# OllieBoyne/sslap

Hardware: AMD Instinct MI355X
Metric: Medges/s (bid-phase CSR nnz/s) + solve ms, N=200k d=0.1% sparse LAP (higher is better)
Workload: dtype f64

## Files before the change

### sslap_amd/csrc/device_common.hpp

```cpp
#pragma once
#include <hip/hip_runtime.h>
#include <stdint.h>

#include <type_traits>

namespace misslap {

constexpr int kWave = 64;
constexpr int kPosNone = 0x7fffffff;
constexpr int kTailMax = 512;

constexpr int kErrNegativeBid = 1;
constexpr int kErrRowsUnsorted = 2;
constexpr int kErrRowGap = 4;
constexpr int kErrNonFinite = 8;
constexpr int kErrColNegative = 16;
constexpr int kErrLdsBase = 32;
constexpr int kErrTooMany = 64;
constexpr int kErrPriceFell = 128;

struct Ctl {
    int K;
    int nholes;
    int nleft;
// ... 149 lines not shown
}
__device__ __forceinline__ double readlane_f64(double v, int l) {
    const int lo = __builtin_amdgcn_readlane(__double2loint(v), l);
    const int hi = __builtin_amdgcn_readlane(__double2hiint(v), l);
    return __hiloint2double(hi, lo);
}

#define MISSLAP_WAVE_MAX_STEP(T, EXCH) \
    {                                  \
        const T o = EXCH;              \
        v = o > v ? o : v;             \
    }
__device__ __forceinline__ int wave_max_i32(int v) {
    MISSLAP_WAVE_MAX_STEP(int, __builtin_amdgcn_mov_dpp(v, kDppXor1, 0xF, 0xF, true))
    MISSLAP_WAVE_MAX_STEP(int, __builtin_amdgcn_mov_dpp(v, kDppXor2, 0xF, 0xF, true))
    MISSLAP_WAVE_MAX_STEP(int, __builtin_amdgcn_mov_dpp(v, kDppHalfMirror, 0xF, 0xF, true))
    MISSLAP_WAVE_MAX_STEP(int, __builtin_amdgcn_mov_dpp(v, kDppMirror, 0xF, 0xF, true))
    MISSLAP_WAVE_MAX_STEP(int, (dpp_i32<kDppBcast15, 0xA>(v)))
    MISSLAP_WAVE_MAX_STEP(int, (dpp_i32<kDppBcast31, 0xC>(v)))
    return __builtin_amdgcn_readlane(v, 63);
}
__device__ __forceinline__ double wave_max_f64(double v) {
    v = __builtin_fmax(v, dpp_f64<kDppXor1>(v));
    v = __builtin_fmax(v, dpp_f64<kDppXor2>(v));
    v = __builtin_fmax(v, dpp_f64<kDppHalfMirror>(v));
    v = __builtin_fmax(v, dpp_f64<kDppMirror>(v));
    v = __builtin_fmax(v, (dpp_f64<kDppBcast15, 0xA>(v)));
    v = __builtin_fmax(v, (dpp_f64<kDppBcast31, 0xC>(v)));
    return readlane_f64(v, 63);
}
#undef MISSLAP_WAVE_MAX_STEP

struct Top2 {
    double v, w;
    int g;
};
__device__ __forceinline__ Top2 top2_wave_reduce(const Top2 &x) {
    Top2 r;
    r.v = wave_max_f64(x.v);
    r.g = wave_max_i32(x.v == r.v ? x.g : -1);
    r.w = wave_max_f64(x.g == r.g ? x.w : x.v);
    return r;
}

struct __attribute__((aligned(16))) PriceRec {
    double price;
    int owner;
    int ostart;
};

__device__ __forceinline__ int lane_id() { return threadIdx.x & (kWave - 1); }
__device__ __forceinline__ unsigned long long lanemask_lt() {
    return (1ull << lane_id()) - 1ull;
}

constexpr int kCandLanes = 32;
constexpr int kCandMax = 30;
constexpr int kCandMin = 24;
constexpr int kCandRowMax = 4 * kWave;

template <int CTRL>
__device__ __forceinline__ int dppf_i32(int v) {
    return __builtin_amdgcn_mov_dpp(v, CTRL, 0xF, 0xF, true);
}
template <int CTRL>
__device__ __forceinline__ double dppf_f64(double v) {
    return __hiloint2double(dppf_i32<CTRL>(__double2hiint(v)), dppf_i32<CTRL>(__double2loint(v)));
}
__device__ __forceinline__ double half_max_f64(double v) {
    v = __builtin_fmax(v, dppf_f64<kDppXor1>(v));
    v = __builtin_fmax(v, dppf_f64<kDppXor2>(v));
    v = __builtin_fmax(v, dppf_f64<kDppHalfMirror>(v));
    v = __builtin_fmax(v, dppf_f64<kDppMirror>(v));
    v = __builtin_fmax(v, (dpp_f64<kDppBcast15, 0xA>(v)));
    return v;
}
__device__ __forceinline__ int half_max_i32(int v) {
    v = max(v, dppf_i32<kDppXor1>(v));
    v = max(v, dppf_i32<kDppXor2>(v));
    v = max(v, dppf_i32<kDppHalfMirror>(v));
    v = max(v, dppf_i32<kDppMirror>(v));
    v = max(v, (dpp_i32<kDppBcast15, 0xA>(v)));
    return v;
}

__device__ __forceinline__ double slot_cost(const int2 &s) { return (double)__int_as_float(s.y); }
__device__ __forceinline__ double slot_cost(const Slot64 &s) { return s.c; }
__device__ __forceinline__ double slot_cost_at(const int2 &s, int sl) {
    return (double)__int_as_float(__builtin_amdgcn_readlane(s.y, sl));
}
__device__ __forceinline__ double slot_cost_at(const Slot64 &s, int sl) { return readlane_f64(s.c, sl); }
template <class Slot>
struct LineIO;
template <>
struct LineIO<int2> {
    static __device__ __forceinline__ int2 load(const int2 *cand, const double *, size_t idx) { return cand[idx]; }
    static __device__ __forceinline__ int2 make(int x, int y) { return make_int2(x, y); }
};
template <>
struct LineIO<Slot64> {
    static __device__ __forceinline__ Slot64 load(const int2 *cand, const double *cost, size_t idx) {
        const int2 s = cand[idx];
        Slot64 r;
        r.x = s.x;
        r.y = s.y;
        r.c = cost[idx];
        return r;
    }
    static __device__ __forceinline__ Slot64 make(int x, int y) {
        Slot64 r;
        r.x = x;
        r.y = y;
        r.c = 0.0;
        return r;
    }
};

struct CandBid {
    bool hit;
    unsigned long long key;
    int obj;
    int prev, pstart;
    int len;
};

struct RecSource {
    const PriceRec *rec;
    __device__ __forceinline__ PriceRec get(int col) const { return rec[col]; }
};
struct PriceSource {
    const double *price;
    __device__ __forceinline__ PriceRec get(int col) const {
        PriceRec r;
        r.price = price[col];
        r.owner = -1;
        r.ostart = 0;
        return r;
    }
};

template <class Slot, class Src>
__device__ __forceinline__ PriceRec cand_gather2(const Slot slot, const bool act0, const bool act1, const Src &src) {
    const int lane = lane_id(), l32 = lane & (kCandLanes - 1);
    const bool active = lane < kCandLanes ? act0 : act1;
    const bool is_cand = active & (l32 >= 1) & (l32 <= kCandMax) & (slot.x >= 0);
    return src.get(is_cand ? slot.x : 0);
}
template <class Slot, class Early, class S = NoStamp>
__device__ __forceinline__ void cand_eval2_r(Slot &slot, const PriceRec r, const bool act0, const bool act1,
                                             const double eps, CandBid (&out)[2], int &err, Early &&early,
                                             const S &stamp = S(), int *alive = nullptr);
template <class Slot, class Src, class Early, class S = NoStamp>
__device__ __forceinline__ void cand_eval2(Slot &slot, const bool act0, const bool act1, const Src &src,
                                           const double eps, CandBid (&out)[2], int &err, Early &&early,
                                           const S &stamp = S(), int *alive = nullptr) {
    stamp(1);
    const PriceRec r = cand_gather2(slot, act0, act1, src);
    stamp(2);
    cand_eval2_r(slot, r, act0, act1, eps, out, err, early, stamp, alive);
}
template <class Slot, class Early, class S>
__device__ __forceinline__ void cand_eval2_r(Slot &slot, const PriceRec r, const bool act0, const bool act1,
                                             const double eps, CandBid (&out)[2], int &err, Early &&early,
                                             const S &stamp, int *alive) {
    const int lane = lane_id(), l32 = lane & (kCandLanes - 1);
    const double ninf = -__builtin_huge_val();
// ... 381 lines not shown
```

### sslap_amd/csrc/host_rounds.hpp

```cpp
#pragma once

namespace {
void begin_phase(misslap_solver *h) {
    if (h->cand != nullptr && !h->lines_dropped && (double)h->eps < h->lines_safe_eps) h->lines_dropped = true;
    h->phases_run += 1;
    h->phases_with_lines += h->lines_live() ? 1 : 0;
}

RoundArgs round_args(misslap_solver *h) {
    RoundArgs a;
    a.ctl = h->ctl;
    a.row_ptr = h->row_ptr;
    a.price = h->price;
    a.rec = h->rec;
    a.p2o = h->p2o;
    a.o2p = h->o2p;
    a.U = h->U;
    a.bid_key = h->bid_key;
    a.bid_obj = h->bid_obj;
    a.bid_rec = h->bid_rec;
    a.best_key = h->best_key;
    a.best_pos = h->best_pos;
    a.cnt = h->cnt;
    a.hole_list = h->hole_list;
// ... 355 lines not shown
    if (h->round_small) {
        h->round_small = false;
        h->K_exact = false;
        MISSLAP_LAUNCH(h, k_round_small, (F_k_round_small), 1024, dim3(1), dim3(1024), a);
        HIP_TRY(hipGetLastError());
        return MISSLAP_OK;
    }
    h->K_exact = false;
    h->round_ordered = false;
    if ((h->world == 1 || h->K_ub < h->shard_min_K) && (long long)h->K_ub * h->apply_bidders_ratio <= h->n_cols)
        MISSLAP_LAUNCH(h, k_apply_bidders, (F_k_apply_bidders), 256, dim3(blocks_for(h->K_ub, 256)), dim3(256), a);
    else
        MISSLAP_LAUNCH(h, k_apply, (F_k_apply), 256, dim3(blocks_for(h->n_cols, 256)), dim3(256), a);
    if (h->K_ub <= kCompactSmallMax) {
        MISSLAP_LAUNCH(h, k_compact_small, (F_k_compact_small), 1024, dim3(1), dim3(1024), a);
    } else {
        const int cb = blocks_for(h->K_ub, kChunk);
        MISSLAP_LAUNCH(h, k_compact_count, (F_k_compact_count), 256, dim3(cb), dim3(256), a);
        MISSLAP_LAUNCH(h, k_compact_scatter, (F_k_compact_scatter), 256, dim3(cb), dim3(256), a);
        MISSLAP_LAUNCH(h, k_compact_fill, (F_k_compact_fill), 256, dim3(blocks_for(h->K_ub, 256)), dim3(256), a);
    }
    HIP_TRY(hipGetLastError());
    return MISSLAP_OK;
}

int launch_tail(misslap_solver *h) {
    if (h->thr <= 0) return MISSLAP_OK;
    h->ctl_fresh = false;
    h->untouched = false;
    const long long long_after = std::max<long long>(kLongRowsAfterTailRoundsMin, h->n_rows / 64);
    if (h->long_rows_later && h->tail_rounds_host >= long_after) {
        h->long_rows = true;
        h->long_rows_later = false;
    }
    TailArgs a;
    a.ctl = h->ctl;
    a.row_ptr = h->row_ptr;
    a.price = h->price;
    a.rec = h->rec;
    a.p2o = h->p2o;
    a.o2p = h->o2p;
    a.U = h->U;
    const bool lines = h->lines_live();
    a.cand = lines ? h->cand : nullptr;
    a.cand64 = lines ? h->cand64 : nullptr;
    a.round_budget = h->long_rows && lines && h->line_maintenance ? h->tail_round_budget
                     : h->long_rows_later                            ? (int)std::min<long long>(std::max<long long>(long_after, 1), 1 << 30)
                                                                     : 0;
    if (a.round_budget == 0 || a.round_budget > h->tail_launch_rounds) a.round_budget = h->tail_launch_rounds;
    a.thr = h->thr;
    a.eps = h->eps;
    ProfRec *pr = nullptr;
    if (h->profile) {
        pr = prof_next(h, 1);
        if (!pr) return fail(MISSLAP_ERR_HIP, "hipEventCreate failed");
        HIP_TRY(hipEventRecord(pr->start, h->stream));
    }
    const EdgesF32 e32{h->edges32};
    const EdgesF64 e64{h->col, h->val64};
    const int long_max = !(lines && h->line_maintenance && h->long_rows) ? 0 : (h->max_row_len <= 256 * kLongPer ? 256 : 512) * kLongPer;
    const int min_alive_long = kLongRowMinAlive;
    const bool in_batch = h->batch != nullptr;
    if (in_batch) h->batch->hold_next = true;
#define MISSLAP_LAUNCH_TAIL(E, ED)                                                                                       \
    do {                                                                                                                 \
        if (lines && h->line_maintenance)                                                                                \
            MISSLAP_LAUNCH(h, k_refresh_lines<E>, (F_k_refresh_lines<E>), kBidBlock,                                     \
                           dim3(blocks_for((h->n_rows + 1) / 2, kBidBlock / kWave)), dim3(kBidBlock), round_args(h), ED, \
                           (int)kCandMaintenanceMin, long_max, min_alive_long);                                          \
        if (lines && h->line_maintenance && h->long_rows) {                                                              \
            if (h->max_row_len <= 256 * kLongPer)                                                                        \
                MISSLAP_LAUNCH(h, (k_refresh_long<E, 256>), (F_k_refresh_long<E, 256>), 256, dim3(blocks_for(h->n_rows, 1)), \
                               dim3(256), round_args(h), ED);                                                            \
            else                                                                                                         \
                MISSLAP_LAUNCH(h, (k_refresh_long<E, 512>), (F_k_refresh_long<E, 512>), 512, dim3(blocks_for(h->n_rows, 1)), \
                               dim3(512), round_args(h), ED);                                                            \
        }                                                                                                                \
        if (h->K_ub > kTeamMax || in_batch)                                                                              \
            MISSLAP_LAUNCH(h, (k_tail<E, 2 * kTailMax>), (F_k_tail<E, 2 * kTailMax, false>), 2 * kTailMax, dim3(1),      \
                           dim3(2 * kTailMax), a, ED);                                                                   \
        if ((h->K_ub > 2 || in_batch) && lines)                                                                          \
            MISSLAP_LAUNCH(h, (k_tail<E, 2 * kTailMax, true>), (F_k_tail<E, 2 * kTailMax, true>), 2 * kTailMax, dim3(1), \
                           dim3(2 * kTailMax), a, ED);                                                                   \
        if (lines) MISSLAP_LAUNCH(h, (k_tail<E, 2 * kWave>), (F_k_tail<E, 2 * kWave, false>), 2 * kWave, dim3(1),        \
                                  dim3(2 * kWave), a, ED);                                                               \
        else MISSLAP_LAUNCH(h, (k_tail<E, kTailMax>), (F_k_tail<E, kTailMax, false>), kTailMax, dim3(1), dim3(kTailMax), a, ED); \
    } while (0)
    if (h->f32) MISSLAP_LAUNCH_TAIL(EdgesF32, e32);
    else MISSLAP_LAUNCH_TAIL(EdgesF64, e64);
#undef MISSLAP_LAUNCH_TAIL
    if (pr) HIP_TRY(hipEventRecord(pr->stop, h->stream));
    h->live_valid = !h->live_off && h->live_dev != nullptr;
    MISSLAP_LAUNCH(h, k_sync_from_rec, (F_k_sync_from_rec), 256, dim3(blocks_for(h->n_cols, 256)), dim3(256), h->ctl,
                   (const PriceRec *)h->rec, h->price, h->o2p, h->p2o, (const int *)h->U, h->n_cols,
                   (h->cand != nullptr && !h->lines_dropped) ? 1 : 0, h->live_valid ? h->live_dev : (unsigned long long *)nullptr,
                   ++h->ticket);
    HIP_TRY(hipGetLastError());
    h->phase_fresh = false;
    if (h->tail_nits0 < 0) h->tail_nits0 = h->h_ctl->nits;
    return MISSLAP_OK;
}

int check_lanes(const misslap_solver *h) {
    if (!h->tiled_ok) return 0;
    const int *shp = kTiledShapes[h->tiled_shape];
    return (shp[3] == 2 && shp[4] == kTileColsHalf) ? shp[6] : 0;
}
#define MISSLAP_FOR_CHECK_LANES(X) X(4) X(8) X(16)
#define MISSLAP_CHECK_KERNEL(GL) k_bid_tiled<1024, 4, 2, 2, kTileColsHalf, 3, 0, GL, 1, 1>
#define MISSLAP_CHECK_KERNEL_FMT(GL, FMT) k_bid_tiled<1024, 4, 2, 2, kTileColsHalf, 3, 0, GL, 1, 1, FMT>

size_t final_pass_grid_max(size_t n_rows, int n_cus) {
    const size_t per_wg_min = (size_t)((1024 - 64 * 3) / 16) * 4;
    return std::max<size_t>((n_rows + per_wg_min - 1) / per_wg_min, (size_t)n_cus);
}
int launch_rows_gather(misslap_solver *h, float eps, const FinalOut &fo, int n_rows, int *n_blocks = nullptr) {
    const int grid = blocks_for(n_rows, 4);
    if (n_blocks) *n_blocks = grid;
    if (h->f32) {
        EdgesF32 ed{h->edges32};
        MISSLAP_LAUNCH(h, k_ece<EdgesF32>, (F_k_ece<EdgesF32>), 256, dim3(grid), dim3(256), h->ctl, ed, (const int *)h->row_ptr,
                       (const double *)h->price, (const int *)h->p2o, n_rows, eps, fo);
    } else {
        EdgesF64 ed{h->col, h->val64};
        MISSLAP_LAUNCH(h, k_ece<EdgesF64>, (F_k_ece<EdgesF64>), 256, dim3(grid), dim3(256), h->ctl, ed, (const int *)h->row_ptr,
                       (const double *)h->price, (const int *)h->p2o, n_rows, eps, fo);
    }
    HIP_TRY(hipGetLastError());
    return MISSLAP_OK;
}
int launch_rows_all(misslap_solver *h, float eps, const FinalOut &fo, int *n_blocks = nullptr) {
    const int gl = check_lanes(h);
    if (!gl) return launch_rows_gather(h, eps, fo, h->n_rows, n_blocks);
    RoundArgs a = round_args(h);
    a.eps = eps;
    a.launch_edges = nullptr;
    TiledArgs ta{h->tiled, h->tcol, h->seg4, h->T, 0, h->n_tiled,
                 nullptr, nullptr, h->ovf_ptr, h->ovf_q, h->ovf_cap, nullptr, nullptr, h->n_rows, nullptr, fo};
    const int groups = (1024 - 64 * 3) / gl, per_wg_max = groups * 4;
    long long grid = ((long long)h->n_rows + per_wg_max - 1) / per_wg_max;
    const long long spread = std::min<long long>(h->n_cus, ((long long)h->n_rows + groups - 1) / groups);
    if (grid < spread) grid = spread;
    if (fo.fin && grid > h->fin_slots_n) return fail(MISSLAP_ERR_STATE, "final pass: grid %lld exceeds its result slots (%d)", grid, h->fin_slots_n);
    if (n_blocks) *n_blocks = (int)grid;
    const size_t lds = tiled_lds_bytes(kTileColsHalf);
    if (h->tiled_fmt == 0) {
        switch (gl) {
#define X(GL) \
    case GL: MISSLAP_LAUNCH_PLAIN(h, (MISSLAP_CHECK_KERNEL(GL)), dim3((unsigned)grid), dim3(1024), lds, a, ta); break;
            MISSLAP_FOR_CHECK_LANES(X)
#undef X
        }
    } else {
        switch (h->tiled_fmt * 100 + gl) {
#define X(FMT, GL) \
    case FMT * 100 + GL: MISSLAP_LAUNCH_PLAIN(h, (MISSLAP_CHECK_KERNEL_FMT(GL, FMT)), dim3((unsigned)grid), dim3(1024), lds, a, ta); break;
            MISSLAP_FOR_FMT_LANES(X)
#undef X
        }
    }
    HIP_TRY(hipGetLastError());
    return MISSLAP_OK;
}

int run_ece(misslap_solver *h, float eps, int *ok) {
    int rc = read_status(h);
    if (rc) return rc;
    if (h->h_ctl->K > 0) {
// ... 48 lines not shown
```

### sslap_amd/csrc/kernels_tail.hpp

```cpp
#pragma once
#include "device_common.hpp"

namespace misslap {

struct TailArgs {
    Ctl *ctl;
    const int *row_ptr;
    double *price;
    PriceRec *rec;
    int *p2o;
    int *o2p;
    int *U;
    int2 *cand;
    double *cand64;
    int thr;
    int round_budget;
    float eps;
};

constexpr int kHashSize = 2048;

__device__ __forceinline__ unsigned long long readlane_u64(unsigned long long v, int l) {
    const int lo = __builtin_amdgcn_readlane((int)(unsigned)(v & 0xffffffffull), l);
    const int hi = __builtin_amdgcn_readlane((int)(unsigned)(v >> 32), l);
// ... 190 lines not shown
    K = pi != -1;
    nits += r;
#ifdef MISSLAP_TAIL_STAMP
    if (lane == 0) {
        for (int k = 1; k <= 6; ++k) a.ctl->dbg[5 + k] += sacc[k];
    }
#endif
}

template <class E>
__device__ __forceinline__ void tail_solo_mode(const TailArgs &a, const E &ed, int *sU, int *sStart, int &K,
                                               long long &nits, const long long max_iter, const double eps,
                                               TailStats &st) {
    const int lane = lane_id();
    int pi[2], ps[2];
    pi[0] = __builtin_amdgcn_readfirstlane(sU[0]);
    ps[0] = __builtin_amdgcn_readfirstlane(sStart[0]);
    pi[1] = K > 1 ? __builtin_amdgcn_readfirstlane(sU[1]) : -1;
    ps[1] = K > 1 ? __builtin_amdgcn_readfirstlane(sStart[1]) : 0;
    if (K == 1) {
        tail_chain_mode(a, ed, pi[0], ps[0], K, nits, max_iter, eps, st);
        if (lane == 0) {
            sU[0] = pi[0];
            sU[1] = -1;
            sStart[0] = ps[0];
        }
        return;
    }
    TwoFetch<E> tf;
    tf.slot = cand_no_line<typename E::Slot>();
    request_two(a, ed, pi[0], ps[0], pi[1], ps[1], tf);
#ifdef MISSLAP_TAIL_STAMP_SOLO
    unsigned long long sacc[8] = {0, 0, 0, 0, 0, 0, 0, 0}, sprev = __builtin_amdgcn_s_memtime();
    const CycleStamp stamp{sacc, &sprev, true};
#else
    const NoStamp stamp;
#endif
    for (;;) {
        CandBid b[2];
        CandBuildArgs bd;
        int bd_person;
        int sp[2] = {-2, -2};
        bid_two(a, ed, pi, ps, tf, eps, b, bd, bd_person, st, [&](const CandBid(&w)[2]) {
            sp[0] = pi[0] >= 0 ? w[0].prev : -1;
            sp[1] = pi[1] >= 0 ? w[1].prev : -1;
            request_two(a, ed, sp[0], 0, sp[1], 0, tf);
        }, stamp);
        stamp.light(5);
        nits += 1;
        bool win0 = true, win1 = pi[1] >= 0;
        if (win1 && b[0].obj == b[1].obj) {
            if (b[1].key > b[0].key) win0 = false;
            else win1 = false;
        }
        if (lane == 0) {
            if (win0) apply_winner(a, pi[0], ps[0], b[0].obj, b[0].prev, b[0].key);
            if (win1) apply_winner(a, pi[1], ps[1], b[1].obj, b[1].prev, b[1].key);
        }
        if (win0) {
            pi[0] = b[0].prev;
            ps[0] = b[0].pstart;
        }
        if (win1) {
            pi[1] = b[1].prev;
            ps[1] = b[1].pstart;
        }
        if (pi[0] == -1 && pi[1] != -1) {
            pi[0] = pi[1];
            ps[0] = ps[1];
            pi[1] = -1;
        }
        K = (pi[0] != -1) + (pi[1] != -1);
        const bool done = K <= 1 || nits >= max_iter;
        if (!done && (sp[0] != pi[0] || sp[1] != pi[1])) request_two(a, ed, pi[0], ps[0], pi[1], ps[1], tf);
        if (bd_person >= 0) tail_build(a, bd_person, bd, eps, st);
        stamp.light(6);
        if (done) break;
    }
    if (K == 1 && nits < max_iter) tail_chain_mode(a, ed, pi[0], ps[0], K, nits, max_iter, eps, st);
#ifdef MISSLAP_TAIL_STAMP_SOLO
    if (lane == 0)
        for (int k = 1; k <= 6; ++k) a.ctl->dbg[5 + k] += sacc[k];
#endif
    if (lane == 0) {
        sU[0] = pi[0];
        sU[1] = pi[1];
        sStart[0] = ps[0];
        sStart[1] = ps[1];
    }
}

constexpr int kTeamMax = 16;
constexpr int kTeamTab = 64;
__device__ __forceinline__ void tail_barrier_lds() { asm volatile("s_waitcnt lgkmcnt(0)\n\ts_barrier" ::: "memory"); }

template <class E>
__device__ __forceinline__ void tail_team_mode(const TailArgs &a, const E &ed, int *sU, int *sStart, int &K,
                                               long long &nits, const long long max_iter, const double eps,
                                               TailStats &st) {
    const int lane = lane_id(), wave = __builtin_amdgcn_readfirstlane(threadIdx.x >> 6);
    static_assert(kTeamMax <= 2 * (kTailMax / kWave) && kTeamMax <= kWave, "two list slots per wavefront");
    __shared__ unsigned long long tKey[2][kTeamMax];
    __shared__ int tObj[2][kTeamMax], tPrev[2][kTeamMax], tPst[2][kTeamMax], tU[2][kTeamMax], tS[2][kTeamMax];
    __shared__ int wTab[kTailMax / kWave][kTeamTab];
    const int n0 = 2 * wave;
    int pi[2], ps[2];
#pragma unroll
    for (int X = 0; X < 2; ++X) {
        pi[X] = n0 + X < K ? __builtin_amdgcn_readfirstlane(sU[min(n0 + X, kTailMax - 1)]) : -1;
        ps[X] = n0 + X < K ? __builtin_amdgcn_readfirstlane(sStart[min(n0 + X, kTailMax - 1)]) : 0;
    }
    wTab[wave][lane & (kTeamTab - 1)] = -1;
    TwoFetch<E> tf;
    tf.slot = cand_no_line<typename E::Slot>();
    if (n0 < K) request_two(a, ed, pi[0], ps[0], pi[1], ps[1], tf);
    __syncthreads();
#ifdef MISSLAP_TAIL_STAMP_TEAM
    unsigned long long sacc[8] = {0, 0, 0, 0, 0, 0, 0, 0}, sprev = __builtin_amdgcn_s_memtime();
    const CycleStamp stamp{sacc, &sprev, wave == 0};
#else
    const NoStamp stamp;
#endif
    int par = 0;
    for (;;) {
        int sp[2] = {-2, -2};
        CandBuildArgs bd;
        int bd_person = -1;
        stamp.light(0);
        if (n0 < K) {
            CandBid b[2];
            bid_two(a, ed, pi, ps, tf, eps, b, bd, bd_person, st, [&](const CandBid(&w)[2]) {
                sp[0] = pi[0] >= 0 ? w[0].prev : -1;
                sp[1] = pi[1] >= 0 ? w[1].prev : -1;
                request_two(a, ed, sp[0], 0, sp[1], 0, tf);
            });
            if (lane == 0) {
#pragma unroll
                for (int X = 0; X < 2; ++X)
                    if (pi[X] >= 0) {
                        tKey[par][n0 + X] = b[X].key;
                        tObj[par][n0 + X] = b[X].obj;
                        tPrev[par][n0 + X] = b[X].prev;
                        tPst[par][n0 + X] = b[X].pstart;
                        tU[par][n0 + X] = pi[X];
                        tS[par][n0 + X] = ps[X];
                    }
            }
        }
        stamp.light(1);
        tail_barrier_lds();
        stamp.light(2);
        {
            const bool act = lane < K;
            const int ls = min(lane, kTeamMax - 1);
            const unsigned long long lkey = act ? tKey[par][ls] : 0ull;
            const int lobj = act ? tObj[par][ls] : (-2 - lane);
            const int lprev = act ? tPrev[par][ls] : 0, lpst = act ? tPst[par][ls] : 0;
            int u = act ? tU[par][ls] : -1;
            int sx = act ? tS[par][ls] : 0;
            int hs = 0;
            bool dup = false;
            if (act) {
                hs = (int)(((unsigned)lobj * 2654435761u) >> 26) & (kTeamTab - 1);
                for (;;) {
                    const int old = atomicCAS(&wTab[wave][hs], -1, lobj);
                    if (old == -1) break;
// ... 1 lines not shown
                        dup = true;
                        break;
                    }
                    hs = (hs + 1) & (kTeamTab - 1);
                }
            }
            const bool contested = __any(dup);
            if (act && !dup) wTab[wave][hs] = -1;
            const bool ends = __any(act && lprev == -1);
#ifdef MISSLAP_TAIL_STAMP_TEAM
            if (threadIdx.x == 0) sacc[5] += (!contested && !ends), sacc[6] += contested, sacc[7] += 1;
#endif
            if (!contested && !ends) {
                if (act && n0 < K) apply_winner(a, u, sx, lobj, lprev, lkey);
#pragma unroll
                for (int X = 0; X < 2; ++X) {
                    const int w = __builtin_amdgcn_readlane(lprev, min(n0 + X, kWave - 1));
                    const int ws = __builtin_amdgcn_readlane(lpst, min(n0 + X, kWave - 1));
                    pi[X] = n0 + X < K ? w : -1;
                    ps[X] = n0 + X < K ? ws : 0;
                }
            } else {
                bool lose = false;
                for (int m = 0; m < K; ++m) {
                    const int om = __builtin_amdgcn_readlane(lobj, m);
                    const bool same = (om == lobj) && (m != lane);
                    if (__any(same)) {
                        const unsigned long long km = readlane_u64(lkey, m);
                        lose |= same && (km > lkey || (km == lkey && m < lane));
                    }
                }
                const bool won = act && !lose;
                if (won && n0 < K) apply_winner(a, u, sx, lobj, lprev, lkey);
                u = won ? lprev : u;
                sx = won ? lpst : sx;
                const unsigned long long kmask = (1ull << K) - 1ull;
                const unsigned long long holes = __ballot(act && u == -1) & kmask;
                const int Kn = K - __popcll(holes);
                const unsigned long long lmask = (1ull << Kn) - 1ull;
                unsigned long long hl = holes & lmask;
                unsigned long long mv = ~holes & ~lmask & kmask;
                while (hl) {
                    const int hk = __ffsll((long long)hl) - 1, mk = __ffsll((long long)mv) - 1;
                    const int mu = __builtin_amdgcn_readlane(u, mk), ms = __builtin_amdgcn_readlane(sx, mk);
                    if (lane == hk) {
                        u = mu;
                        sx = ms;
                    }
                    hl &= hl - 1;
                    mv &= mv - 1;
                }
                K = Kn;
#pragma unroll
                for (int X = 0; X < 2; ++X) {
                    pi[X] = n0 + X < K ? __builtin_amdgcn_readlane(u, min(n0 + X, kWave - 1)) : -1;
                    ps[X] = n0 + X < K ? __builtin_amdgcn_readlane(sx, min(n0 + X, kWave - 1)) : 0;
                }
            }
        }
        stamp.light(3);
        par ^= 1;
        nits += 1;
        const bool done = K <= 2 || nits >= max_iter;
        if (!done && n0 < K && (sp[0] != pi[0] || sp[1] != pi[1]))
            request_two(a, ed, pi[0], ps[0], pi[1], ps[1], tf);
        if (bd_person >= 0) tail_build(a, bd_person, bd, eps, st);
        stamp.light(4);
        if (done) break;
    }
#ifdef MISSLAP_TAIL_STAMP_TEAM
    if (threadIdx.x == 0)
        for (int k = 1; k <= 6; ++k) a.ctl->dbg[5 + k] += sacc[k];
#endif
    if (lane < 2 && n0 + lane < kTeamMax) {
        sU[n0 + lane] = lane == 0 ? pi[0] : pi[1];
        sStart[n0 + lane] = lane == 0 ? ps[0] : ps[1];
    }
    __syncthreads();
}

constexpr int kPipeTab = 4096;
__device__ __forceinline__ int pipe_hash(int obj) { return (int)(((unsigned)obj * 2654435761u) >> 20); }
static_assert((1 << 12) == kPipeTab, "pipe_hash keeps the top 12 bits");
__device__ __forceinline__ void patch_rec(PriceRec &r, const bool take, const PriceRec &nw) {
    r.price = take ? nw.price : r.price;
    r.owner = take ? nw.owner : r.owner;
    r.ostart = take ? nw.ostart : r.ostart;
}
struct __attribute__((aligned(16))) PipeSlot {
    PriceRec rec;
    int4 aux;
};
struct __attribute__((aligned(16))) PipeLds {
    PipeSlot slot[2][kTeamMax];
    int dirty[2];
    int pad[2];
    int tab[kPipeTab];
};

__device__ __forceinline__ void touch_slot(const int2 &s) { asm volatile("" ::"v"(s.x), "v"(s.y)); }
__device__ __forceinline__ void touch_slot(const Slot64 &s) { asm volatile("" ::"v"(s.x), "v"(s.y), "v"(s.c)); }

template <class E>
__device__ __forceinline__ bool tail_team1_pipe(const TailArgs &a, const E &ed, int *sU, int *sStart, int &K,
                                                long long &nits, const long long max_iter, const double eps,
                                                TailStats &st) {
    const int lane = lane_id(), l32 = lane & (kCandLanes - 1);
    const int wave = __builtin_amdgcn_readfirstlane(threadIdx.x >> 6);
    __shared__ PipeLds L;
    const RecSource src{a.rec};
    const bool cls = (lane >= 1) & (lane <= kCandMax);
    const int n0 = wave;
    int pi = n0 < K ? __builtin_amdgcn_readfirstlane(sU[min(n0, kTailMax - 1)]) : -1;
    int ps = n0 < K ? __builtin_amdgcn_readfirstlane(sStart[min(n0, kTailMax - 1)]) : 0;
    for (int h = threadIdx.x; h < kPipeTab; h += blockDim.x) L.tab[h] = -1;
    if (threadIdx.x < 2) L.dirty[threadIdx.x] = -1;
    typename E::Slot slot = cand_no_line<typename E::Slot>();
    auto request = [&](int person) { slot = line_of<E>(a, person, l32); };
    if (n0 < K) request(pi);
    __syncthreads();
#ifdef MISSLAP_TAIL_STAMP_TEAM
    unsigned long long sacc[8] = {0, 0, 0, 0, 0, 0, 0, 0}, sprev = __builtin_amdgcn_s_memtime();
    const CycleStamp stamp{sacc, &sprev, wave == 0};
#else
    const NoStamp stamp;
#endif
    const int rmax = round_limit(nits, max_iter);
    int r = 0;
    int par = 0;
    const int ls = min(lane, kTeamMax - 1);
    PriceRec grec = PriceRec{0.0, -1, 0};
    bool have_g = false;
    for (;;) {
        if (n0 >= K) {
            if (lane == 0) {
                sU[n0] = -1;
                sStart[n0] = 0;
            }
            tail_barrier_lds();
            nits += r;
            return true;
        }
        int sp = -2;
        CandBid b;
        b.hit = false;
        stamp.light(0);
        if (!have_g) grec = cand_gather1(slot, cls, src);
#ifdef MISSLAP_TAIL_STAMP_TEAM
        asm volatile("s_waitcnt vmcnt(0)" ::: "memory");
        stamp.light(1);
#endif
        cand_eval1_r(slot, grec, cls, eps, b, st.bad_hi, [&](const CandBid &w) {
            sp = w.prev;
            request(sp);
        });
        if (!b.hit) {
            CandBuildArgs bd;
            const typename E::Raw none[4] = {};
            const int e = a.row_ptr[pi + 1 + lane_zero()];
            wave_bid_full<E, RecSource, true, false>(ed, src, ps, e, none, eps, b, bd, st.err);
            st.misses += 1;
            st.miss_edges += (unsigned long long)b.len;
            if (bd.want) tail_build(a, pi, bd, eps, st);
        }
        st.edges += (unsigned long long)b.len;
        st.bids += 1;
        stamp.light(2);
        if (lane == 0) {
            const int old = atomicExch(&L.tab[pipe_hash(b.obj)], r);
            PriceRec mine;
            mine.price = key_to_bid(b.key);
// ... 8 lines not shown
        stamp.light(4);
        {
            const int dflag = L.dirty[par];
            const PriceRec lrec = L.slot[par][ls].rec;
            const int lobj = L.slot[par][ls].aux.x;
#ifdef MISSLAP_TAIL_STAMP_TEAM
            asm volatile("s_waitcnt lgkmcnt(0)" ::: "memory");
            stamp.light(5);
#endif
            if (__builtin_amdgcn_readfirstlane(dflag) != r) {
                have_g = sp == b.prev;
                if (have_g) {
                    touch_slot(slot);
                    if (lane < K) a.rec[lobj] = lrec;
                    grec = cand_gather1(slot, cls, src);
                } else {
                    if (lane < K) a.rec[lobj] = lrec;
                }
                pi = b.prev;
                ps = b.pstart;
            } else {
                have_g = false;
                const bool act = lane < K;
                const int4 laux = L.slot[par][ls].aux;
                const unsigned long long lkey = act ? bid_to_key(lrec.price) : 0ull;
                const int lo = act ? laux.x : (-2 - lane);
                const int lprev = act ? laux.y : 0, lpst = act ? laux.z : 0;
                int u = act ? lrec.owner : -1;
                int sx = act ? lrec.ostart : 0;
                bool lose = false;
                for (int m = 0; m < K; ++m) {
                    const int om = __builtin_amdgcn_readlane(lo, m);
                    const bool same = (om == lo) && (m != lane);
                    if (__any(same)) {
                        const unsigned long long km = readlane_u64(lkey, m);
                        lose |= same && (km > lkey || (km == lkey && m < lane));
                    }
                }
                const bool won = act && !lose;
                if (won) apply_winner(a, u, sx, lo, lprev, lkey);
                u = won ? lprev : u;
                sx = won ? lpst : sx;
                const unsigned long long kmask = (1ull << K) - 1ull;
                const unsigned long long holes = __ballot(act && u == -1) & kmask;
                const int Kn = K - __popcll(holes);
                const unsigned long long lmask = (1ull << Kn) - 1ull;
                unsigned long long hl = holes & lmask;
                unsigned long long mv = ~holes & ~lmask & kmask;
                while (hl) {
                    const int hk = __ffsll((long long)hl) - 1, mk = __ffsll((long long)mv) - 1;
                    const int mu = __builtin_amdgcn_readlane(u, mk), ms = __builtin_amdgcn_readlane(sx, mk);
                    if (lane == hk) {
                        u = mu;
                        sx = ms;
                    }
                    hl &= hl - 1;
                    mv &= mv - 1;
                }
                K = Kn;
                pi = n0 < K ? __builtin_amdgcn_readlane(u, min(n0, kWave - 1)) : -1;
                ps = n0 < K ? __builtin_amdgcn_readlane(sx, min(n0, kWave - 1)) : 0;
            }
        }
        par ^= 1;
        r += 1;
        const bool done = K <= 2 || r >= rmax;
        if (!done && n0 < K && sp != pi) request(pi);
        stamp.light(6);
        if (done) break;
    }
    nits += r;
#ifdef MISSLAP_TAIL_STAMP_TEAM
    if (threadIdx.x == 0)
        for (int k = 1; k <= 6; ++k) a.ctl->dbg[5 + k] += sacc[k];
#endif
    if (lane == 0 && n0 < kTeamMax) {
        sU[n0] = pi;
        sStart[n0] = ps;
    }
    __syncthreads();
    return false;
}

template <class E>
__device__ __forceinline__ void tail_duo_pipe(const TailArgs &a, const E &ed, int *sU, int *sStart, int &K,
                                              long long &nits, const long long max_iter, const double eps,
                                              TailStats &st) {
    const int lane = lane_id(), l32 = lane & (kCandLanes - 1);
    const int w = __builtin_amdgcn_readfirstlane(threadIdx.x >> 6);
    const int o = w ^ 1;
    __shared__ PipeSlot D[2][2];
    const RecSource src{a.rec};
    const bool cls = (lane >= 1) & (lane <= kCandMax);
    int me = __builtin_amdgcn_readfirstlane(sU[w]), mys = __builtin_amdgcn_readfirstlane(sStart[w]);
    typename E::Slot slot = cand_no_line<typename E::Slot>();
    auto request = [&](int person) { slot = line_of<E>(a, person, l32); };
    request(me);
    tail_barrier_lds();
#ifdef MISSLAP_TAIL_STAMP_DUO
    unsigned long long sacc[8] = {0, 0, 0, 0, 0, 0, 0, 0}, sprev = __builtin_amdgcn_s_memtime();
    const CycleStamp stamp{sacc, &sprev, w == 0};
#else
    const NoStamp stamp;
#endif
    const int rmax = round_limit(nits, max_iter);
    int r = 0;
    PriceRec grec = PriceRec{0.0, -1, 0};
    bool have_g = false;
    int par = 0;
    bool pend = false;
    PriceRec prec = PriceRec{0.0, -1, 0};
    int pobj = 0;
    auto flush_store = [&]() {
        if (pend) {
            if (lane < 2) a.rec[pobj] = prec;
            pend = false;
        }
    };
    for (;;) {
        int sp = -2;
        CandBid b;
        b.hit = false;
        stamp.light(0);
        if (!have_g) {
            flush_store();
            grec = cand_gather1(slot, cls, src);
        }
        cand_eval1_r(slot, grec, cls, eps, b, st.bad_hi, [&](const CandBid &x) {
            sp = x.prev;
            request(sp);
        });
        if (!b.hit) {
            flush_store();
            CandBuildArgs bd;
            const typename E::Raw none[4] = {};
            const int e = a.row_ptr[me + 1 + lane_zero()];
            wave_bid_full<E, RecSource, true, false>(ed, src, mys, e, none, eps, b, bd, st.err);
            st.misses += 1;
            st.miss_edges += (unsigned long long)b.len;
            if (bd.want) tail_build(a, me, bd, eps, st);
            b.hit = false;
        }
        flush_store();
        st.edges += (unsigned long long)b.len;
        st.bids += 1;
        stamp.light(1);
        PriceRec mine;
        mine.price = key_to_bid(b.key);
        mine.owner = me;
        mine.ostart = mys;
        if (lane == 0) {
            D[par][w].rec = mine;
            D[par][w].aux = make_int4(b.obj, b.prev, b.pstart, 0);
        }
        have_g = b.hit && b.prev >= 0;
        if (have_g) grec = cand_gather1(slot, cls, src);
        stamp.light(2);
        tail_barrier_lds();
        stamp.light(3);
        const PriceRec orec = D[par][o].rec;
        const int4 oaux = D[par][o].aux;
        r += 1;
        const int unclean = __builtin_amdgcn_readfirstlane((int)(oaux.x == b.obj) | (int)(oaux.y < 0)) | (int)(b.prev < 0);
        if (!unclean) {
            if (have_g) {
                const int c = slot.x;
                patch_rec(grec, c == b.obj, mine);
                patch_rec(grec, c == oaux.x, orec);
            }
            pend = true;
            prec = mine;
            patch_rec(prec, lane == 1, orec);
            pobj = lane == 1 ? oaux.x : b.obj;
            me = b.prev;
            mys = b.pstart;
        } else {
            const unsigned long long okey = bid_to_key(readlane_f64(orec.price, 0));
            const int oobj = __builtin_amdgcn_readfirstlane(oaux.x), oprev = __builtin_amdgcn_readfirstlane(oaux.y);
            const int opst = __builtin_amdgcn_readfirstlane(oaux.z);
            const int ome = __builtin_amdgcn_readfirstlane(orec.owner), omys = __builtin_amdgcn_readfirstlane(orec.ostart);
            int pi[2], ps[2];
            pi[0] = w ? ome : me, pi[1] = w ? me : ome;
            ps[0] = w ? omys : mys, ps[1] = w ? mys : omys;
            const unsigned long long key0 = w ? okey : b.key, key1 = w ? b.key : okey;
            const int obj0 = w ? oobj : b.obj, obj1 = w ? b.obj : oobj;
            const int prev0 = w ? oprev : b.prev, prev1 = w ? b.prev : oprev;
            const int pst0 = w ? opst : b.pstart, pst1 = w ? b.pstart : opst;
            bool win0 = true, win1 = true;
            if (obj0 == obj1) {
                if (key1 > key0) win0 = false;
                else win1 = false;
            }
            if (lane == 0) {
                if (win0) apply_winner(a, pi[0], ps[0], obj0, prev0, key0);
                if (win1) apply_winner(a, pi[1], ps[1], obj1, prev1, key1);
            }
            if (win0) {
                pi[0] = prev0;
                ps[0] = pst0;
            }
            if (win1) {
                pi[1] = prev1;
                ps[1] = pst1;
            }
            if (pi[0] == -1 && pi[1] != -1) {
                pi[0] = pi[1];
                ps[0] = ps[1];
                pi[1] = -1;
            }
            K = (pi[0] != -1) + (pi[1] != -1);
            me = w ? pi[1] : pi[0];
            mys = w ? ps[1] : ps[0];
            have_g = false;
        }
        stamp.light(4);
        par ^= 1;
        const bool done = K <= 1 || r >= rmax;
        if (!done && sp != me) request(me);
        stamp.light(5);
        if (done) break;
    }
    flush_store();
    nits += r;
#ifdef MISSLAP_TAIL_STAMP_DUO
    if (w == 0 && lane == 0)
        for (int k = 1; k <= 5; ++k) a.ctl->dbg[5 + k] += sacc[k];
#endif
    if (lane == 0) {
        sU[w] = me;
        sStart[w] = mys;
    }
    tail_barrier_lds();
}

template <class E, int kThreads, bool kTeamOnly>
__device__ __forceinline__ void k_tail_body(TailArgs a, E ed) {
    static_assert(!kTeamOnly || (kThreads == 2 * kTailMax && kThreads / kWave == kTeamMax), "one slot per wavefront");
    constexpr bool kBlockOnly = kThreads > kTailMax && !kTeamOnly;
    constexpr bool kDuoOnly = kThreads == 2 * kWave;
    static_assert(!kDuoOnly || !kTeamOnly, "roles are exclusive");
    __shared__ int sU[kTailMax];
    __shared__ unsigned long long sKey[kTailMax];
    __shared__ int sObj[kTailMax];
    __shared__ int sPrev[kTailMax];
    __shared__ int sStart[kTailMax];
    __shared__ int sPst[kTailMax];
    __shared__ int sList[kTailMax];
    __shared__ int hObj[kHashSize];
    __shared__ unsigned long long hKey[kHashSize];
    __shared__ int hPos[kHashSize];
    __shared__ int sCnt[3][kThreads / kWave];
    __shared__ int sK, sMissCnt;
    __shared__ long long sNits;

    Ctl *ctl = a.ctl;
    const int t = threadIdx.x, lane = t & 63, wave = t >> 6;
    constexpr int nwaves = kThreads / kWave;
    int K = ctl->K;
    long long nits = ctl->nits;
    const long long max_iter =
        a.round_budget > 0 ? min(ctl->max_iter, nits + (long long)(kBlockOnly ? max(a.round_budget / 4, 1) : a.round_budget))
                           : ctl->max_iter;
    if (K == 0 || K > a.thr || nits >= max_iter) return;
    if (kBlockOnly && K <= kTeamMax) return;
    if (kTeamOnly && (K <= 2 || K > kTeamMax)) return;
    if (kDuoOnly && (K > 2 || !E::kCand || a.cand == nullptr)) return;
    if (!kBlockOnly && !kTeamOnly && a.round_budget > 0 && K > 2 && E::kCand && a.cand != nullptr) return;
    const int K0 = K;
    const long long nits0 = nits;
    for (int n = t; n < kTailMax; n += kThreads) {
        sU[n] = (n < K) ? a.U[n] : -1;
        sStart[n] = (n < K) ? a.row_ptr[sU[n]] : 0;
    }
    if (!kDuoOnly)
        for (int h = t; h < kHashSize; h += kThreads) {
            hObj[h] = -1;
            hKey[h] = 0ull;
            hPos[h] = kPosNone;
        }
    const double eps = (double)a.eps;
    TailStats st;
    st.edges = st.miss_edges = st.builds = 0ull;
    st.bids = st.misses = st.bad_hi = 0u;
    st.err = 0;
    st.hint = 0.0;
    if (t == 0) sMissCnt = 0;
    __syncthreads();

    unsigned long long md[6] = {0, 0, 0, 0, 0, 0};
#ifdef MISSLAP_TAIL_STAMP_BLOCK
    unsigned long long bacc[8] = {0, 0, 0, 0, 0, 0, 0, 0};
#endif
    auto mode_begin = [&](int m) {
        md[3 + m] -= __builtin_amdgcn_s_memrealtime();
        md[m] -= (unsigned long long)nits;
    };
    auto mode_end = [&](int m) {
        md[3 + m] += __builtin_amdgcn_s_memrealtime();
        md[m] += (unsigned long long)nits;
    };
    auto flush_stats = [&]() {
        if (lane == 0) {
            if (st.bids) {
                const unsigned long long hits = (unsigned long long)(st.bids - st.misses), hit_edges = st.edges - st.miss_edges;
                atomicAdd(&ctl->edges, st.edges);
                atomicAdd(&ctl->tail_edges, st.edges);
                atomicAdd(&ctl->bids, (unsigned long long)st.bids);
                if (hits) {
                    atomicAdd(&ctl->cand_hits, hits);
                    atomicAdd(&ctl->cand_edges, hit_edges);
                }
                atomicAdd(&ctl->dbg[12], (unsigned long long)st.bids);
                atomicAdd(&ctl->dbg[13], hits);
                atomicAdd(&ctl->dbg[14], st.builds);
                atomicAdd(&ctl->dbg[15], hit_edges);
            }
            if (bad_hi_is_error(st.bad_hi)) st.err |= kErrNegativeBid;
            if (st.err) atomicOr(&ctl->err, st.err);
        }
    };
    for (;;) {
        if (kBlockOnly && K <= kTeamMax) break;
        if (kDuoOnly) {
            mode_begin(0);
            if (K == 2) tail_duo_pipe(a, ed, sU, sStart, K, nits, max_iter, eps, st);
            if (wave == 1) {
                flush_stats();
                return;
            }
            if (K == 1 && nits < max_iter) {
                int pi = __builtin_amdgcn_readfirstlane(sU[0]), ps = __builtin_amdgcn_readfirstlane(sStart[0]);
                tail_chain_mode(a, ed, pi, ps, K, nits, max_iter, eps, st);
                if (lane == 0) {
                    sU[0] = pi;
                    sU[1] = -1;
                    sStart[0] = ps;
                }
            }
            mode_end(0);
            break;
        }
        if (kTeamOnly) {
            if (K > 2 && nits < max_iter) {
                mode_begin(1);
                if (tail_team1_pipe(a, ed, sU, sStart, K, nits, max_iter, eps, st)) {
                    flush_stats();
                    return;
                }
                mode_end(1);
            }
            break;
        }
        if (!kBlockOnly && !kTeamOnly && K == 2 && K0 <= 2 && E::kCand && a.cand != nullptr) {
            if (wave >= 2) {
                flush_stats();
                return;
            }
            mode_begin(0);
            tail_duo_pipe(a, ed, sU, sStart, K, nits, max_iter, eps, st);
            if (wave == 1) {
                flush_stats();
                return;
            }
            if (K > 0 && nits < max_iter) tail_solo_mode(a, ed, sU, sStart, K, nits, max_iter, eps, st);
            mode_end(0);
            break;
        }
        if (!kBlockOnly && K <= 2) {
            if (wave == 0) {
                mode_begin(0);
                tail_solo_mode(a, ed, sU, sStart, K, nits, max_iter, eps, st);
                mode_end(0);
                if (lane == 0) {
                    sK = K;
                    sNits = nits;
                }
            }
            __syncthreads();
            K = sK;
            nits = sNits;
            break;
        }
        if (!kBlockOnly && K <= kTeamMax) {
            mode_begin(1);
            tail_team_mode(a, ed, sU, sStart, K, nits, max_iter, eps, st);
            mode_end(1);
            if (K == 0 || nits >= max_iter) break;
            continue;
        }
        mode_begin(2);
#ifdef MISSLAP_TAIL_STAMP_BLOCK
        unsigned long long sprev_b = __builtin_amdgcn_s_memtime();
        const CycleStamp bstamp{bacc, &sprev_b, wave == 0};
#else
        const NoStamp bstamp;
#endif
        {
            const RecSource src{a.rec};
            constexpr int kBlockDepth = kBlockOnly ? 1 : 3;
            for (int base = 0; base < K; base += kBlockDepth * 2 * nwaves) {
                typename E::Slot sl[kBlockDepth];
                PriceRec rr[kBlockDepth];
#pragma unroll
                for (int c = 0; c < kBlockDepth; ++c) {
                    const int nme = base + c * 2 * nwaves + 2 * wave + (lane >> 5);
                    const int pme = nme < K ? sU[min(nme, kTailMax - 1)] : -1;
                    sl[c] = cand_no_line<typename E::Slot>();
                    if (E::kCand && a.cand != nullptr) sl[c] = line_of<E>(a, pme, lane & (kCandLanes - 1));
                }
                bstamp(1);
#pragma unroll
                for (int c = 0; c < kBlockDepth; ++c) {
                    const int n0 = base + c * 2 * nwaves + 2 * wave;
                    if (E::kCand) rr[c] = cand_gather2(sl[c], n0 < K, n0 + 1 < K, src);
                }
                bstamp(2);
#pragma unroll
                for (int c = 0; c < kBlockDepth; ++c) {
                    const int n0 = base + c * 2 * nwaves + 2 * wave;
                    if (n0 >= K) continue;
                    CandBid b[2];
                    b[0].hit = b[1].hit = false;
                    if (E::kCand) cand_eval2_r(sl[c], rr[c], n0 < K, n0 + 1 < K, eps, b, st.err, NoEarly());
#pragma unroll
                    for (int X = 0; X < 2; ++X) {
                        const int n = n0 + X;
                        if (n >= K) continue;
                        if (b[X].hit) {
                            if (lane == 0) {
                                sKey[n] = b[X].key;
                                sObj[n] = b[X].obj;
                                sPrev[n] = b[X].prev;
                                sPst[n] = b[X].pstart;
                            }
                            st.edges += (unsigned long long)b[X].len;
                            st.bids += 1;
                        } else if (lane == 0) {
                            sList[atomicAdd(&sMissCnt, 1)] = n;
                        }
                    }
                }
            }
            __syncthreads();
            bstamp(3);
            const int nmiss = sMissCnt;
            for (int m = wave; m < nmiss; m += nwaves) {
                const int n = __builtin_amdgcn_readfirstlane(sList[m]);
                const int i = __builtin_amdgcn_readfirstlane(sU[n]);
// ... 200 lines not shown
```

Baseline: 4754.

## Replace two-wave duo pipeline with single-wave paired tail mode

Replaces the two-wavefront duo tail, which exchanged bids through LDS with barriers each round, with one wavefront that handles both remaining persons in its two 32-lane halves. A fast argmax path uses a new permlane16_swap-based half-wave max with a ballot when each half has a unique maximum. The duo kernel is launched with 64 threads, and the K==2 duo branch in the general kernel is removed. This avoids inter-wave barrier and LDS round trips, but loses the pipelined overlap of gathers and store flushing, and a miss in either half now stalls both.

Result: faster. 4842, median of 6 (+1.9%).

```diff
diff --git a/sslap_amd/csrc/device_common.hpp b/sslap_amd/csrc/device_common.hpp
--- a/sslap_amd/csrc/device_common.hpp
+++ b/sslap_amd/csrc/device_common.hpp
@@ -255,6 +255,14 @@
     v = max(v, dppf_i32<kDppMirror>(v));
     v = max(v, (dpp_i32<kDppBcast15, 0xA>(v)));
     return v;
+}
+__device__ __forceinline__ int half_allmax_i32(int v) {
+    v = max(v, dppf_i32<kDppXor1>(v));
+    v = max(v, dppf_i32<kDppXor2>(v));
+    v = max(v, dppf_i32<kDppHalfMirror>(v));
+    v = max(v, dppf_i32<kDppMirror>(v));
+    const auto s = __builtin_amdgcn_permlane16_swap(v, v, false, false);
+    return max((int)s[0], (int)s[1]);
 }
 
 __device__ __forceinline__ double slot_cost(const int2 &s) { return (double)__int_as_float(s.y); }
diff --git a/sslap_amd/csrc/host_rounds.hpp b/sslap_amd/csrc/host_rounds.hpp
--- a/sslap_amd/csrc/host_rounds.hpp
+++ b/sslap_amd/csrc/host_rounds.hpp
@@ -461,8 +461,7 @@
         if ((h->K_ub > 2 || in_batch) && lines)                                                                          \
             MISSLAP_LAUNCH(h, (k_tail<E, 2 * kTailMax, true>), (F_k_tail<E, 2 * kTailMax, true>), 2 * kTailMax, dim3(1), \
                            dim3(2 * kTailMax), a, ED);                                                                   \
-        if (lines) MISSLAP_LAUNCH(h, (k_tail<E, 2 * kWave>), (F_k_tail<E, 2 * kWave, false>), 2 * kWave, dim3(1),        \
-                                  dim3(2 * kWave), a, ED);                                                               \
+        if (lines) MISSLAP_LAUNCH(h, (k_tail<E, kWave>), (F_k_tail<E, kWave, false>), kWave, dim3(1), dim3(kWave), a, ED); \
         else MISSLAP_LAUNCH(h, (k_tail<E, kTailMax>), (F_k_tail<E, kTailMax, false>), kTailMax, dim3(1), dim3(kTailMax), a, ED); \
     } while (0)
     if (h->f32) MISSLAP_LAUNCH_TAIL(EdgesF32, e32);
diff --git a/sslap_amd/csrc/kernels_tail.hpp b/sslap_amd/csrc/kernels_tail.hpp
--- a/sslap_amd/csrc/kernels_tail.hpp
+++ b/sslap_amd/csrc/kernels_tail.hpp
@@ -296,6 +296,155 @@
     if (lane == 0)
         for (int k = 1; k <= 6; ++k) a.ctl->dbg[5 + k] += sacc[k];
 #endif
+    if (lane == 0) {
+        sU[0] = pi[0];
+        sU[1] = pi[1];
+        sStart[0] = ps[0];
+        sStart[1] = ps[1];
+    }
+}
+
+template <class E>
+__device__ __forceinline__ void tail_pair_mode(const TailArgs &a, const E &ed, int *sU, int *sStart, int &K,
+                                               long long &nits, const long long max_iter, const double eps,
+                                               TailStats &st) {
+    const int lane = lane_id(), l32 = lane & (kCandLanes - 1);
+    const bool upper = lane >= kCandLanes;
+    const RecSource src{a.rec};
+    const bool cls = (l32 >= 1) & (l32 <= kCandMax);
+    const double ninf = -__builtin_huge_val();
+    int pi[2], ps[2];
+#pragma unroll
+    for (int X = 0; X < 2; ++X) {
+        pi[X] = __builtin_amdgcn_readfirstlane(sU[X]);
+        ps[X] = __builtin_amdgcn_readfirstlane(sStart[X]);
+    }
+    typename E::Slot slot;
+    auto request = [&](int p0, int p1) { slot = line_of<E>(a, upper ? p1 : p0, l32); };
+    const int rmax = round_limit(nits, max_iter);
+    int r = 0;
+    if (K == 2) request(pi[0], pi[1]);
+#ifdef MISSLAP_TAIL_STAMP_DUO
+    unsigned long long sacc[8] = {0, 0, 0, 0, 0, 0, 0, 0}, sprev = __builtin_amdgcn_s_memtime();
+    const CycleStamp stamp{sacc, &sprev, true};
+#else
+    const NoStamp stamp;
+#endif
+    while (K == 2) {
+        stamp(1);
+        const PriceRec g = cand_gather1(slot, cls, src);
+        stamp(2);
+        const bool is_cand = cls & (slot.x >= 0);
+        const double v = is_cand ? slot_cost(slot) - g.price : ninf;
+        const int hw = __double2hiint(v);
+        const int k = hw ^ ((hw >> 31) & 0x7fffffff);
+        const unsigned long long eq = __ballot(k == half_allmax_i32(k));
+        const unsigned eq0 = (unsigned)eq, eq1 = (unsigned)(eq >> 32);
+        int G[2];
+        double V[2];
+        if ((int)(__popc(eq0) == 1) & (int)(__popc(eq1) == 1)) {
+            G[0] = __ffs((int)eq0) - 1;
+            G[1] = __ffs((int)eq1) + (kCandLanes - 1);
+            V[0] = readlane_f64(v, G[0]);
+            V[1] = readlane_f64(v, G[1]);
+        } else {
+            const double vm = half_max_f64(v);
+            V[0] = readlane_f64(vm, kCandLanes - 1);
+            V[1] = readlane_f64(vm, kWave - 1);
+            const int gm = half_max_i32((is_cand & (v == (upper ? V[1] : V[0]))) ? lane : -1);
+            G[0] = __builtin_amdgcn_readlane(gm, kCandLanes - 1);
+            G[1] = __builtin_amdgcn_readlane(gm, kWave - 1);
+        }
+        CandBid b[2];
+        double tau[2], c1[2];
+#pragma unroll
+        for (int X = 0; X < 2; ++X) {
+            const int sl = max(G[X], kCandLanes * X);
+            tau[X] = readlane_f64(__hiloint2double(slot.y, slot.x), kCandLanes * X);
+            b[X].len = __builtin_amdgcn_readlane(slot.x, kCandLanes * X + kCandLanes - 1);
+            b[X].obj = __builtin_amdgcn_readlane(slot.x, sl);
+            b[X].prev = __builtin_amdgcn_readlane(g.owner, sl);
+            b[X].pstart = __builtin_amdgcn_readlane(g.ostart, sl);
+            c1[X] = slot_cost_at(slot, sl);
+        }
+        const int sp0 = b[0].prev, sp1 = b[1].prev;
+        request(sp0, sp1);
+        stamp.light(3);
+        const double wm = half_max_f64(((lane == G[0]) | (lane == G[1])) ? ninf : v);
+        const double W[2] = {readlane_f64(wm, kCandLanes - 1), readlane_f64(wm, kWave - 1)};
+#pragma unroll
+        for (int X = 0; X < 2; ++X) {
+            b[X].hit = (G[X] >= 0) & (V[X] > tau[X]) & (W[X] >= tau[X]);
+            const double bid = (c1[X] - W[X]) + eps;
+            st.bad_hi = max(st.bad_hi, b[X].hit ? (unsigned)__double2hiint(bid) : 0u);
+            b[X].key = bid_to_key(bid);
+        }
+        stamp.light(4);
+#pragma unroll
+        for (int X = 0; X < 2; ++X) {
+            if (!b[X].hit) {
+                CandBuildArgs bd;
+                const typename E::Raw none[4] = {};
+                const int e = a.row_ptr[pi[X] + 1];
+                wave_bid_full<E, RecSource, true, false>(ed, src, ps[X], e, none, eps, b[X], bd, st.err);
+                st.misses += 1;
+                st.miss_edges += (unsigned long long)b[X].len;
+                if (bd.want) tail_build(a, pi[X], bd, eps, st);
+            }
+        }
+        stamp.light(5);
+        st.edges += (unsigned long long)(b[0].len + b[1].len);
+        st.bids += 2;
+        r += 1;
+        if ((b[0].obj != b[1].obj) & (b[0].prev >= 0) & (b[1].prev >= 0)) {
+            if (l32 == 0) {
+                PriceRec w;
+                w.price = key_to_bid(upper ? b[1].key : b[0].key);
+                w.owner = upper ? pi[1] : pi[0];
+                w.ostart = upper ? ps[1] : ps[0];
+                a.rec[upper ? b[1].obj : b[0].obj] = w;
+            }
+#pragma unroll
+            for (int X = 0; X < 2; ++X) {
+                pi[X] = b[X].prev;
+                ps[X] = b[X].pstart;
+            }
+        } else {
+            bool win0 = true, win1 = true;
+            if (b[0].obj == b[1].obj) {
+                if (b[1].key > b[0].key) win0 = false;
+                else win1 = false;
+            }
+            if (lane == 0) {
+                if (win0) apply_winner(a, pi[0], ps[0], b[0].obj, b[0].prev, b[0].key);
+                if (win1) apply_winner(a, pi[1], ps[1], b[1].obj, b[1].prev, b[1].key);
+            }
+            if (win0) {
+                pi[0] = b[0].prev;
+                ps[0] = b[0].pstart;
+            }
+            if (win1) {
+                pi[1] = b[1].prev;
+                ps[1] = b[1].pstart;
+            }
+            if (pi[0] == -1 && pi[1] != -1) {
+                pi[0] = pi[1];
+                ps[0] = ps[1];
+                pi[1] = -1;
+            }
+            K = (pi[0] != -1) + (pi[1] != -1);
+        }
+        const bool done = K <= 1 || r >= rmax;
+        if (!done && (sp0 != pi[0] || sp1 != pi[1])) request(pi[0], pi[1]);
+        stamp.light(6);
+        if (done) break;
+    }
+    nits += r;
+#ifdef MISSLAP_TAIL_STAMP_DUO
+    if (lane == 0)
+        for (int k = 1; k <= 6; ++k) a.ctl->dbg[5 + k] += sacc[k];
+#endif
+    if (K == 1 && nits < max_iter) tail_chain_mode(a, ed, pi[0], ps[0], K, nits, max_iter, eps, st);
     if (lane == 0) {
         sU[0] = pi[0];
         sU[1] = pi[1];
@@ -463,11 +612,6 @@
 constexpr int kPipeTab = 4096;
 __device__ __forceinline__ int pipe_hash(int obj) { return (int)(((unsigned)obj * 2654435761u) >> 20); }
 static_assert((1 << 12) == kPipeTab, "pipe_hash keeps the top 12 bits");
-__device__ __forceinline__ void patch_rec(PriceRec &r, const bool take, const PriceRec &nw) {
-    r.price = take ? nw.price : r.price;
-    r.owner = take ? nw.owner : r.owner;
-    r.ostart = take ? nw.ostart : r.ostart;
-}
 struct __attribute__((aligned(16))) PipeSlot {
     PriceRec rec;
     int4 aux;
@@ -642,162 +786,11 @@
     return false;
 }
 
-template <class E>
-__device__ __forceinline__ void tail_duo_pipe(const TailArgs &a, const E &ed, int *sU, int *sStart, int &K,
-                                              long long &nits, const long long max_iter, const double eps,
-                                              TailStats &st) {
-    const int lane = lane_id(), l32 = lane & (kCandLanes - 1);
-    const int w = __builtin_amdgcn_readfirstlane(threadIdx.x >> 6);
-    const int o = w ^ 1;
-    __shared__ PipeSlot D[2][2];
-    const RecSource src{a.rec};
-    const bool cls = (lane >= 1) & (lane <= kCandMax);
-    int me = __builtin_amdgcn_readfirstlane(sU[w]), mys = __builtin_amdgcn_readfirstlane(sStart[w]);
-    typename E::Slot slot = cand_no_line<typename E::Slot>();
-    auto request = [&](int person) { slot = line_of<E>(a, person, l32); };
-    request(me);
-    tail_barrier_lds();
-#ifdef MISSLAP_TAIL_STAMP_DUO
-    unsigned long long sacc[8] = {0, 0, 0, 0, 0, 0, 0, 0}, sprev = __builtin_amdgcn_s_memtime();
-    const CycleStamp stamp{sacc, &sprev, w == 0};
-#else
-    const NoStamp stamp;
-#endif
-    const int rmax = round_limit(nits, max_iter);
-    int r = 0;
-    PriceRec grec = PriceRec{0.0, -1, 0};
-    bool have_g = false;
-    int par = 0;
-    bool pend = false;
-    PriceRec prec = PriceRec{0.0, -1, 0};
-    int pobj = 0;
-    auto flush_store = [&]() {
-        if (pend) {
-            if (lane < 2) a.rec[pobj] = prec;
-            pend = false;
-        }
-    };
-    for (;;) {
-        int sp = -2;
-        CandBid b;
-        b.hit = false;
-        stamp.light(0);
-        if (!have_g) {
-            flush_store();
-            grec = cand_gather1(slot, cls, src);
-        }
-        cand_eval1_r(slot, grec, cls, eps, b, st.bad_hi, [&](const CandBid &x) {
-            sp = x.prev;
-            request(sp);
-        });
-        if (!b.hit) {
-            flush_store();
-            CandBuildArgs bd;
-            const typename E::Raw none[4] = {};
-            const int e = a.row_ptr[me + 1 + lane_zero()];
-            wave_bid_full<E, RecSource, true, false>(ed, src, mys, e, none, eps, b, bd, st.err);
-            st.misses += 1;
-            st.miss_edges += (unsigned long long)b.len;
-            if (bd.want) tail_build(a, me, bd, eps, st);
-            b.hit = false;
-        }
-        flush_store();
-        st.edges += (unsigned long long)b.len;
-        st.bids += 1;
-        stamp.light(1);
-        PriceRec mine;
-        mine.price = key_to_bid(b.key);
-        mine.owner = me;
-        mine.ostart = mys;
-        if (lane == 0) {
-            D[par][w].rec = mine;
-            D[par][w].aux = make_int4(b.obj, b.prev, b.pstart, 0);
-        }
-        have_g = b.hit && b.prev >= 0;
-        if (have_g) grec = cand_gather1(slot, cls, src);
-        stamp.light(2);
-        tail_barrier_lds();
-        stamp.light(3);
-        const PriceRec orec = D[par][o].rec;
-        const int4 oaux = D[par][o].aux;
-        r += 1;
-        const int unclean = __builtin_amdgcn_readfirstlane((int)(oaux.x == b.obj) | (int)(oaux.y < 0)) | (int)(b.prev < 0);
-        if (!unclean) {
-            if (have_g) {
-                const int c = slot.x;
-                patch_rec(grec, c == b.obj, mine);
-                patch_rec(grec, c == oaux.x, orec);
-            }
-            pend = true;
-            prec = mine;
-            patch_rec(prec, lane == 1, orec);
-            pobj = lane == 1 ? oaux.x : b.obj;
-            me = b.prev;
-            mys = b.pstart;
-        } else {
-            const unsigned long long okey = bid_to_key(readlane_f64(orec.price, 0));
-            const int oobj = __builtin_amdgcn_readfirstlane(oaux.x), oprev = __builtin_amdgcn_readfirstlane(oaux.y);
-            const int opst = __builtin_amdgcn_readfirstlane(oaux.z);
-            const int ome = __builtin_amdgcn_readfirstlane(orec.owner), omys = __builtin_amdgcn_readfirstlane(orec.ostart);
-            int pi[2], ps[2];
-            pi[0] = w ? ome : me, pi[1] = w ? me : ome;
-            ps[0] = w ? omys : mys, ps[1] = w ? mys : omys;
-            const unsigned long long key0 = w ? okey : b.key, key1 = w ? b.key : okey;
-            const int obj0 = w ? oobj : b.obj, obj1 = w ? b.obj : oobj;
-            const int prev0 = w ? oprev : b.prev, prev1 = w ? b.prev : oprev;
-            const int pst0 = w ? opst : b.pstart, pst1 = w ? b.pstart : opst;
-            bool win0 = true, win1 = true;
-            if (obj0 == obj1) {
-                if (key1 > key0) win0 = false;
-                else win1 = false;
-            }
-            if (lane == 0) {
-                if (win0) apply_winner(a, pi[0], ps[0], obj0, prev0, key0);
-                if (win1) apply_winner(a, pi[1], ps[1], obj1, prev1, key1);
-            }
-            if (win0) {
-                pi[0] = prev0;
-                ps[0] = pst0;
-            }
-            if (win1) {
-                pi[1] = prev1;
-                ps[1] = pst1;
-            }
-            if (pi[0] == -1 && pi[1] != -1) {
-                pi[0] = pi[1];
-                ps[0] = ps[1];
-                pi[1] = -1;
-            }
-            K = (pi[0] != -1) + (pi[1] != -1);
-            me = w ? pi[1] : pi[0];
-            mys = w ? ps[1] : ps[0];
-            have_g = false;
-        }
-        stamp.light(4);
-        par ^= 1;
-        const bool done = K <= 1 || r >= rmax;
-        if (!done && sp != me) request(me);
-        stamp.light(5);
-        if (done) break;
-    }
-    flush_store();
-    nits += r;
-#ifdef MISSLAP_TAIL_STAMP_DUO
-    if (w == 0 && lane == 0)
-        for (int k = 1; k <= 5; ++k) a.ctl->dbg[5 + k] += sacc[k];
-#endif
-    if (lane == 0) {
-        sU[w] = me;
-        sStart[w] = mys;
-    }
-    tail_barrier_lds();
-}
-
 template <class E, int kThreads, bool kTeamOnly>
 __device__ __forceinline__ void k_tail_body(TailArgs a, E ed) {
     static_assert(!kTeamOnly || (kThreads == 2 * kTailMax && kThreads / kWave == kTeamMax), "one slot per wavefront");
     constexpr bool kBlockOnly = kThreads > kTailMax && !kTeamOnly;
-    constexpr bool kDuoOnly = kThreads == 2 * kWave;
+    constexpr bool kDuoOnly = kThreads == kWave;
     static_assert(!kDuoOnly || !kTeamOnly, "roles are exclusive");
     __shared__ int sU[kTailMax];
     __shared__ unsigned long long sKey[kTailMax];
@@ -883,20 +876,7 @@
         if (kBlockOnly && K <= kTeamMax) break;
         if (kDuoOnly) {
             mode_begin(0);
-            if (K == 2) tail_duo_pipe(a, ed, sU, sStart, K, nits, max_iter, eps, st);
-            if (wave == 1) {
-                flush_stats();
-                return;
-            }
-            if (K == 1 && nits < max_iter) {
-                int pi = __builtin_amdgcn_readfirstlane(sU[0]), ps = __builtin_amdgcn_readfirstlane(sStart[0]);
-                tail_chain_mode(a, ed, pi, ps, K, nits, max_iter, eps, st);
-                if (lane == 0) {
-                    sU[0] = pi;
-                    sU[1] = -1;
-                    sStart[0] = ps;
-                }
-            }
+            tail_pair_mode(a, ed, sU, sStart, K, nits, max_iter, eps, st);
             mode_end(0);
             break;
         }
@@ -909,21 +889,6 @@
                 }
                 mode_end(1);
             }
-            break;
-        }
-        if (!kBlockOnly && !kTeamOnly && K == 2 && K0 <= 2 && E::kCand && a.cand != nullptr) {
-            if (wave >= 2) {
-                flush_stats();
-                return;
-            }
-            mode_begin(0);
-            tail_duo_pipe(a, ed, sU, sStart, K, nits, max_iter, eps, st);
-            if (wave == 1) {
-                flush_stats();
-                return;
-            }
-            if (K > 0 && nits < max_iter) tail_solo_mode(a, ed, sU, sStart, K, nits, max_iter, eps, st);
-            mode_end(0);
             break;
         }
         if (!kBlockOnly && K <= 2) {
```
